# jmhb0/view_neti

Hardware: AMD Instinct MI355X
Metric: TI train steps/sec (SD-1.5 512^2 bs=4 per GPU) (higher is better)
Workload: dtype f16; 1 GPU; learnable_mode 0, sd15 shapes, 512x512 fp16, bs=4/GPU, grad_accum 1, full train step (VAE+16xCLIP+UNet fwd/bwd+AdamW); global_batch=4, parallelism=dp1, rccl_ranks=1, hipgraph=True

## Files before the change

include/vneti.h:

```cpp
#ifndef VNETI_H
#define VNETI_H
#include <stddef.h>
#include <stdint.h>

#ifdef __cplusplus
extern "C" {
#endif

#define VNETI_ABI_VERSION 1

int vneti_version(void);
int vneti_precision(void);
int vneti_last_error(char* buf, size_t n);

typedef struct vneti_gemm_desc {
  const void* A;
  const void* B;
  void* C;
  long long lda, ldb, ldc;
  int M, N, K;
  int batch;
  long long strideA, strideB, strideC;
  const float* bias;
  const void* rowadd;
// ... 1 lines not shown
  int rows_per_group;
  const void* resid;
  long long ldr;
  float alpha;
  int act;
  int out_f32;
  int conv_mode;
  int Hi, Wi, Ci, Ho, Wo, stride, pad_t, pad_l, ups;
  long long ldx;
  int tile_hint;
  void* workspace;
  long long workspace_bytes;
  int split_k;
  const void* gate_src;
  long long ld_gate;
  int gate_act;
  void* C2;
  long long ldc2;
  int act2;
  void* gn_sums;
  int gn_hw, gn_cpg, gn_groups, gn_slots;
  int geglu;
  int conv_korder;
} vneti_gemm_desc;

int vneti_gemm_f16(const vneti_gemm_desc* d, void* stream);
int vneti_gemm_select_tile(int M, int N, int batch);
int vneti_gemm_select_split(int M, int N, int K, int batch, int tile_hint, long long workspace_bytes);

int vneti_im2col3x3_small(const void* x, int x_is_f32, long long sb, long long sc, long long sy,
                          long long sx, void* out, int Bn, int C, int Hi, int Wi, int Ho, int Wo,
                          int stride, int pad_t, int pad_l, void* stream);

int vneti_conv3x3_in(const void* x, int x_is_f32, long long sb, long long sc, long long sy, long long sx,
                     const void* w_packed, const float* bias, void* out, long long ldo, int Bn, int C, int H, int W,
                     int Co, void* gn_sums, int gn_groups, int gn_slots, void* stream);

int vneti_transpose_f16(const void* in, long long ld_in, long long stride_in, void* out,
                        long long ld_out, long long stride_out, int rows, int cols, int batch,
                        void* stream);
#define VNETI_TRANSPOSE_MAX 4
typedef struct vneti_transpose_desc {
  const void* inp;
  long long ld_in, stride_in;
  void* out;
  long long ld_out, stride_out;
// ... 194 lines not shown
```

view_neti_amd/csrc/gemm_args.h:

```cpp
#pragma once
#include "common.h"

namespace {

struct GemmArgs {
  const half_t* A;
  const half_t* B;
  void* C;
  const float* bias;
  const half_t* rowadd;
  const void* resid;
  float* ws;
  const half_t* gate_src;
  half_t* C2;
  long long ld_gate, ldc2;
  int gate_act, act2;
  float* gn_sums;
  int gn_hw, gn_cpg, gn_G, gn_slots;
  int geglu;
  long long lda, ldb, ldc, ld_rowadd, ldr;
  long long strideA, strideB, strideC;
  uint32_t a_bytes, b_bytes;
  int M, N, K;
  int rows_per_group;
  float alpha;
  int act;
  int out_f32;
  int batch, ksplit, kt_per_split;
  int conv_mode;
  int Hi, Wi, Ci, Ho, Wo, stride, pad_t, pad_l, ups;
  int ldx2;
  int korder;
  int tiles_m, tiles_n;
};

__device__ __forceinline__ float apply_act(float v, int act) {
  switch (act) {
    case 1: return vn_silu(v);
    case 2: return vn_quick_gelu(v);
    case 3: return vn_gelu_erf(v);
    default: return v;
  }
}
__device__ __forceinline__ float act_grad(float f, int act) {
  if (act == 2) {
    float s = vn_sigmoid(1.702f * f);
    return s * (1.f + 1.702f * f * (1.f - s));
  } else if (act == 3) {
    return vn_gelu_erf_grad(f);
  }
  float s = vn_sigmoid(f);
  return s * (1.f + f * (1.f - s));
}

__device__ __forceinline__ int lds_off(int row, int chunk) {
  return row * 128 + ((chunk ^ ((row >> 1) & 7)) << 4);
}
// ... 13 lines not shown
```

view_neti_amd/csrc/gemm_conv.hip:

```cpp
#include "common.h"
#include "gemm_args.h"
#include "../../include/vneti.h"

namespace {

template <int BM, int BN, int WM, int WN, bool F32OUT, bool DMA, int NSTG = 2, int EPI = 2, bool CONV = true>
__global__ __launch_bounds__((BM / WM) * (BN / WN) * 64) void gemm_kernel(
    const half_t* pA, const half_t* pB, uint32_t p_a_bytes, uint32_t p_b_bytes, int p_lda, int p_ldb, int pM, int pN, int pK,
    int p_tiles_m, int p_tiles_n, int p_split_conv , const GemmArgs gfull) {
  GemmArgs g = gfull;
  g.A = pA;
  g.B = pB;
  g.a_bytes = p_a_bytes;
  g.b_bytes = p_b_bytes;
  g.lda = p_lda;
  g.ldb = p_ldb;
  g.M = pM;
  g.N = pN;
  g.K = pK;
  g.tiles_m = p_tiles_m;
  g.tiles_n = p_tiles_n;
  g.kt_per_split = p_split_conv & 0xffff;
  g.ksplit = (p_split_conv >> 16) & 0xff;
  g.conv_mode = p_split_conv >> 24;
  static_assert(NSTG == 2 || ((NSTG == 3 || NSTG == 4) && DMA), "the LDS rings are LDS-DMA only");
  const half_t* const e_gate = EPI == 2 ? g.gate_src : nullptr;
  half_t* const e_C2 = EPI == 2 ? g.C2 : nullptr;
  const int e_geglu = EPI == 2 ? g.geglu : 0;
  const int e_act = EPI == 2 ? g.act : 0;
  float* const e_gn_sums = EPI >= 1 ? g.gn_sums : nullptr;
  const half_t* const e_rowadd = EPI >= 1 ? g.rowadd : nullptr;
  const int e_conv = CONV ? g.conv_mode : 0;
  constexpr int NWM = BM / WM, NWN = BN / WN;
  constexpr int NT = NWM * NWN * 64;
  constexpr int RSTEP = NT / 8;
  constexpr int A_IT = BM / RSTEP, B_IT = BN / RSTEP;
  constexpr int STAGE_BYTES = (BM + BN) * 128;
  constexpr int CS_LD = F32OUT ? (BN + 4) : (BN + 8);
  constexpr int CS_BYTES = BM * CS_LD * (F32OUT ? 4 : 2);
  constexpr int LDS_BYTES = (NSTG * STAGE_BYTES > CS_BYTES) ? NSTG * STAGE_BYTES : CS_BYTES;
  constexpr int GN_IMG = 5, GN_NG = BN / 4 + 2;
  constexpr int GN_BYTES = (F32OUT || EPI == 0) ? 0 : GN_IMG * GN_NG * 4 * 8;
  __shared__ __attribute__((aligned(16))) char smem[LDS_BYTES + GN_BYTES];

  const int tid = threadIdx.x;
  const int lane = tid & 63;
  const int wave = __builtin_amdgcn_readfirstlane(tid >> 6);
  const int wm0 = (wave / NWN) * WM;
  const int wn0 = (wave % NWN) * WN;

  int nblk = g.tiles_m * g.tiles_n;
  int bid = blockIdx.x;
  {
    int q = nblk >> 3, r = nblk & 7, xcd = bid & 7, idx = bid >> 3;
    bid = (xcd < r ? xcd * (q + 1) : r * (q + 1) + (xcd - r) * q) + idx;
  }
  const int tile_m = bid / g.tiles_n;
  const int tile_n = bid - tile_m * g.tiles_n;
  const int m0 = tile_m * BM;
  const int n0 = tile_n * BN;
  const int bz = blockIdx.y;
  const int kz = blockIdx.z;

  const half_t* Ab = g.A + (long long)bz * g.strideA;
  const half_t* Bb = g.B + (long long)bz * g.strideB;
  __amdgpu_buffer_rsrc_t rsA = vn_make_rsrc(Ab, g.a_bytes);
  __amdgpu_buffer_rsrc_t rsB = vn_make_rsrc(Bb, g.b_bytes);

  const int lrow = tid >> 3;
  const int gchunk = DMA ? ((tid & 7) ^ ((lrow >> 1) & 7)) : (tid & 7);

  const float rcp_hw = CONV ? __builtin_amdgcn_rcpf((float)(g.Ho * g.Wo)) : 0.f, rcp_wo = CONV ? __builtin_amdgcn_rcpf((float)g.Wo) : 0.f;
  int a_off[A_IT];
  int a_py[A_IT], a_px[A_IT], a_bh[A_IT];
#pragma unroll
  for (int i = 0; i < A_IT; ++i) {
    int m = m0 + lrow + RSTEP * i;
    bool ok = m < g.M;
    if (e_conv == 0) {
      a_off[i] = ok ? (int)((long long)m * g.lda * 2) + gchunk * 16 : -1;
      a_py[i] = a_px[i] = a_bh[i] = 0;
    } else {
      int rem, ox;
      const int b = vn_divmod(m, g.Ho * g.Wo, rcp_hw, rem);
      const int oy = vn_divmod(rem, g.Wo, rcp_wo, ox);
      a_bh[i] = ok ? b * g.Hi : -1;
      if (e_conv == 1) {
        a_py[i] = oy * g.stride - g.pad_t;
        a_px[i] = ox * g.stride - g.pad_l;
      } else {
        a_py[i] = oy + g.pad_t;
        a_px[i] = ox + g.pad_l;
      }
      a_off[i] = ((b * g.Hi + a_py[i]) * g.Wi + a_px[i]) * g.ldx2 + gchunk * 16;
    }
  }
  int b_off[B_IT];
#pragma unroll
  for (int i = 0; i < B_IT; ++i) {
    int n = n0 + lrow + RSTEP * i;
    b_off[i] = (n < g.N) ? (int)((long long)n * g.ldb * 2) + gchunk * 16 : -1;
  }

  u32x4 ra[DMA ? 1 : A_IT], rb[DMA ? 1 : B_IT];

  auto a_offset = [&](int i, int k0, int dy, int dx, int tapoff) -> uint32_t {
    if (e_conv == 0) return a_off[i] < 0 ? VN_OOB : (uint32_t)(a_off[i] + k0 * 2);
    bool ok = a_bh[i] >= 0;
    if (e_conv == 1 && !g.ups) {
      int iy = a_py[i] + dy, ix = a_px[i] + dx;
      ok = ok && (unsigned)iy < (unsigned)g.Hi && (unsigned)ix < (unsigned)g.Wi;
      return ok ? (uint32_t)(a_off[i] + tapoff) : VN_OOB;
    }
    int iy, ix;
    if (e_conv == 1) {
// ... 18 lines not shown
  };

  uint32_t a_cur[A_IT], b_cur[B_IT];
#pragma unroll
  for (int i = 0; i < B_IT; ++i) b_cur[i] = b_off[i] < 0 ? VN_OOB : (uint32_t)b_off[i];

  auto issue = [&](int kt, int stage, bool first) {
    const int k0 = kt * 64;
    bool recompute = first;
    int dy = 0, dx = 0, tapoff = 0;
    if (e_conv != 0) {
      int tap, ci0;
      if (g.korder) {
        const int chunk = kt / 9;
        tap = kt - chunk * 9;
        ci0 = chunk << 6;
        recompute = true;
      } else {
        tap = k0 / g.Ci;
        ci0 = k0 - tap * g.Ci;
        recompute = recompute || ci0 == 0;
      }
      if (recompute) {
        dy = tap / 3;
        dx = tap - dy * 3;
        tapoff = (e_conv == 1 && !g.ups) ? ((dy * g.Wi + dx) * g.ldx2 + ci0 * 2) : (ci0 * 2 + gchunk * 16);
      }
    }
    if (recompute) {
#pragma unroll
      for (int i = 0; i < A_IT; ++i) a_cur[i] = a_offset(i, k0, dy, dx, tapoff);
      if (first) {
#pragma unroll
        for (int i = 0; i < B_IT; ++i) b_cur[i] += (uint32_t)k0 * 2;
      }
    }
    if constexpr (DMA) {
      char* As = smem + stage * STAGE_BYTES;
      char* Bs = As + BM * 128;
#pragma unroll
      for (int i = 0; i < A_IT; ++i) dma16(rsA, As + (wave * 8 + RSTEP * i) * 128, a_cur[i]);
#pragma unroll
      for (int i = 0; i < B_IT; ++i) dma16(rsB, Bs + (wave * 8 + RSTEP * i) * 128, b_cur[i]);
    } else {
#pragma unroll
      for (int i = 0; i < A_IT; ++i) ra[i] = vn_buf_load16(rsA, a_cur[i]);
#pragma unroll
      for (int i = 0; i < B_IT; ++i) rb[i] = vn_buf_load16(rsB, b_cur[i]);
// ... 238 lines not shown
          q_hi += __shfl_xor(q_hi, off);
        }
      }
      if (gn_img >= 0 && (!uni || lane < CPR)) {
        vn_u64* a = gacc + ((gn_img - gn_img0) * GN_NG + (gn_glo - gn_g0t)) * 4;
        vn_fx_add2(a, s_lo, q_lo);
        if (gn_split < 8) vn_fx_add2(a + 4, s_hi, q_hi);
      }
      s_lo = q_lo = s_hi = q_hi = 0.f;
    };
    for (int idx = tid; idx < BM * CPR; idx += NT) {
      int r = idx / CPR, c = (idx - r * CPR) * 8;
      int m = m0 + r, n = n0 + c;
      const bool valid = m < g.M && n < g.N;
      if (gn) {
        int gn_rem;
        const int img = valid ? vn_divmod(m, g.gn_hw, rcp_gnhw, gn_rem) : gn_img;
        if (__any(img != gn_img)) {
          gn_flush();
          gn_img = img;
        }
      }
      if (!valid) continue;
      half8 v = as_half8(*reinterpret_cast<const u32x4*>(smem + ((size_t)r * CS_LD + c) * 2));
      int ra_rem;
      const half_t* radd = e_rowadd ? e_rowadd + (long long)vn_divmod(m, g.rows_per_group, rcp_rpg, ra_rem) * g.ld_rowadd + n : nullptr;
      if (n + 8 <= g.N) {
        if (radd) {
          half8 t = *reinterpret_cast<const half8*>(radd);
          v = vn_add8(v, t);
        }
        if (Rb) {
          half8 rr = *reinterpret_cast<const half8*>(Rb + (long long)m * g.ldr + n);
          v = vn_add8(v, rr);
        }
        if (e_geglu == 2) {
          const half_t* pp = e_gate + (long long)m * g.ld_gate + 2 * n;
#pragma unroll
          for (int c2 = 0; c2 < 2; ++c2) {
            const half8 pre = *reinterpret_cast<const half8*>(pp + 8 * c2);
            half8 o;
#pragma unroll
            for (int e = 0; e < 4; ++e) {
              const float d = (float)v[4 * c2 + e], hh = (float)pre[e], gg = (float)pre[4 + e];
              float cdf, xpdf;
              vn_gelu_parts(gg, cdf, xpdf);
              o[e] = (half_t)(d * gg * cdf);
              o[4 + e] = (half_t)(d * hh * (cdf + xpdf));
            }
            vn_st16_wt(rsC, (uint32_t)(((long long)m * g.ldc + 2 * n + 8 * c2) * 2), o);
          }
          continue;
        }
        if (e_gate) {
          half8 pre = *reinterpret_cast<const half8*>(e_gate + (long long)m * g.ld_gate + n);
#pragma unroll
          for (int e = 0; e < 8; ++e) v[e] = (half_t)((float)v[e] * act_grad((float)pre[e], g.gate_act));
        }
        if (e_geglu == 1 || (e_C2 && e_geglu == 0)) vn_st16_wt_saved(rsC, (uint32_t)(((long long)m * g.ldc + n) * 2), v);
        else vn_st16_wt(rsC, (uint32_t)(((long long)m * g.ldc + n) * 2), v);
        if (e_geglu == 1) {
          half4 o2;
#pragma unroll
          for (int e = 0; e < 4; ++e) o2[e] = (half_t)((float)v[e] * vn_gelu_erf((float)v[4 + e]));
          *reinterpret_cast<half4*>(e_C2 + (long long)m * g.ldc2 + (n >> 1)) = o2;
        }
        if (gn) {
#pragma unroll
          for (int e = 0; e < 8; ++e) {
            const float x = (float)v[e];
            if (e < gn_split) {
              s_lo += x;
              q_lo += x * x;
            } else {
              s_hi += x;
              q_hi += x * x;
            }
          }
        }
        if (e_C2 && e_geglu == 0) {
          half8 o2;
#pragma unroll
          for (int e = 0; e < 8; ++e) o2[e] = (half_t)apply_act((float)v[e], g.act2);
          vn_st16_wt(rsC2, (uint32_t)(((long long)m * g.ldc2 + n) * 2), o2);
        }
      } else {
        for (int e = 0; e < 8 && n + e < g.N; ++e) {
          float x = (float)v[e];
          if (radd) x = (float)(half_t)(x + (float)radd[e]);
          if (Rb) x = (float)(half_t)(x + (float)Rb[(long long)m * g.ldr + n + e]);
          if (e_gate) x = (float)(half_t)(x * act_grad((float)e_gate[(long long)m * g.ld_gate + n + e], g.gate_act));
          Cb[(long long)m * g.ldc + n + e] = (half_t)x;
          if (e_C2) e_C2[(long long)m * g.ldc2 + n + e] = (half_t)apply_act((float)(half_t)x, g.act2);
          if (gn) {
            const float xs = (float)(half_t)x;
            if (e < gn_split) {
              s_lo += xs;
              q_lo += xs * xs;
            } else {
              s_hi += xs;
              q_hi += xs * xs;
            }
          }
        }
      }
    }
    if (gn) {
      gn_flush();
      __syncthreads();
      const int slot = tile_m % g.gn_slots;
      for (int i = tid; i < GN_IMG * GN_NG; i += NT) {
        const vn_u64* src = gacc + 4 * i;
        if ((src[0] | src[1] | src[2] | src[3]) == 0) continue;
        const int img = gn_img0 + i / GN_NG, grp = gn_g0t + i % GN_NG;
        vn_u64* dst = reinterpret_cast<vn_u64*>(e_gn_sums) + (((long long)img * g.gn_slots + slot) * g.gn_G + grp) * 4;
// ... 10 lines not shown
  GemmArgs g = gfull;
  g.ws = p_ws;
  g.C = pC;
  g.bias = p_bias;
  g.resid = p_resid;
  g.rowadd = p_rowadd;
  g.M = pM;
  g.N = pN;
  g.batch = p_batch;
  g.ksplit = p_ksplit;
  g.ldc = p_ldc;
  g.ldr = p_ldr;
  const unsigned n4 = (unsigned)(g.N + 3) / 4;
  const unsigned gid = blockIdx.x * 256u + threadIdx.x;
  const unsigned total = (unsigned)g.batch * (unsigned)g.M * n4;
  if (gid >= total) return;
  const unsigned row = gid / n4;
  const int c = (int)(gid - row * n4) * 4;
  const int bz = g.batch > 1 ? (int)(row / (unsigned)g.M) : 0;
  const int m = (int)(row - (unsigned)bz * (unsigned)g.M);
  const int ne = min(4, g.N - c);
  const long long zstride = (long long)g.batch * g.M * g.N;
  const float* p0 = g.ws + ((long long)bz * g.M + m) * g.N + c;
  if ((g.N & 3) == 0 && ((g.ldc | g.ldr | g.ld_rowadd | g.ld_gate | g.ldc2) & 3) == 0) {
    const long long co = (long long)bz * g.strideC + (long long)m * g.ldc + c;
    const long long ro = (long long)bz * g.strideC + (long long)m * g.ldr + c;
    f32x4 bv = {0.f, 0.f, 0.f, 0.f}, rf = {0.f, 0.f, 0.f, 0.f};
    half4 rh = {0, 0, 0, 0}, ra = {0, 0, 0, 0}, gt = {0, 0, 0, 0};
    if (g.bias) bv = *reinterpret_cast<const f32x4*>(g.bias + c);
    if (g.resid) {
      if (g.out_f32) rf = *reinterpret_cast<const f32x4*>(reinterpret_cast<const float*>(g.resid) + ro);
      else rh = *reinterpret_cast<const half4*>(reinterpret_cast<const half_t*>(g.resid) + ro);
    }
    if (g.rowadd) ra = *reinterpret_cast<const half4*>(g.rowadd + (long long)(m / g.rows_per_group) * g.ld_rowadd + c);
    if (g.gate_src) gt = *reinterpret_cast<const half4*>(g.gate_src + (long long)m * g.ld_gate + c);
    f32x4 v = {0.f, 0.f, 0.f, 0.f};
    int z = 0;
    for (; z + 4 <= g.ksplit; z += 4) {
      const f32x4 t0 = *reinterpret_cast<const f32x4*>(p0 + (z + 0) * zstride);
      const f32x4 t1 = *reinterpret_cast<const f32x4*>(p0 + (z + 1) * zstride);
      const f32x4 t2 = *reinterpret_cast<const f32x4*>(p0 + (z + 2) * zstride);
      const f32x4 t3 = *reinterpret_cast<const f32x4*>(p0 + (z + 3) * zstride);
      v += t0;
      v += t1;
      v += t2;
      v += t3;
    }
    for (; z < g.ksplit; ++z) v += *reinterpret_cast<const f32x4*>(p0 + z * zstride);
// ... 15 lines not shown
        float y = (float)(half_t)x[e];
        if (g.rowadd) y = (float)(half_t)(y + (float)ra[e]);
        if (g.resid) y = (float)(half_t)(y + (float)rh[e]);
        if (g.gate_src) y = (float)(half_t)(y * act_grad((float)gt[e], g.gate_act));
        o[e] = (half_t)y;
        o2[e] = (half_t)apply_act((float)(half_t)y, g.act2);
      }
      *reinterpret_cast<half4*>(reinterpret_cast<half_t*>(g.C) + co) = o;
      if (g.C2) *reinterpret_cast<half4*>(g.C2 + (long long)m * g.ldc2 + c) = o2;
    }
    return;
  }
  float v[4] = {0.f, 0.f, 0.f, 0.f};
  for (int z = 0; z < g.ksplit; ++z) {
    const float* p = p0 + z * zstride;
    for (int e = 0; e < ne; ++e) v[e] += p[e];
  }
  for (int e = 0; e < ne; ++e) {
    float x = v[e] * g.alpha;
    if (g.bias) x += g.bias[c + e];
    x = apply_act(x, g.act);
    if (g.out_f32) {
      if (g.resid) x += reinterpret_cast<const float*>(g.resid)[(long long)bz * g.strideC + (long long)m * g.ldr + c + e];
      reinterpret_cast<float*>(g.C)[(long long)bz * g.strideC + (long long)m * g.ldc + c + e] = x;
    } else {
      x = (float)(half_t)x;
      if (g.rowadd) x = (float)(half_t)(x + (float)g.rowadd[(long long)(m / g.rows_per_group) * g.ld_rowadd + c + e]);
      if (g.resid)
        x = (float)(half_t)(x + (float)reinterpret_cast<const half_t*>(g.resid)[(long long)bz * g.strideC + (long long)m * g.ldr + c + e]);
      if (g.gate_src) x = (float)(half_t)(x * act_grad((float)g.gate_src[(long long)m * g.ld_gate + c + e], g.gate_act));
      reinterpret_cast<half_t*>(g.C)[(long long)bz * g.strideC + (long long)m * g.ldc + c + e] = (half_t)x;
      if (g.C2) g.C2[(long long)m * g.ldc2 + c + e] = (half_t)apply_act((float)(half_t)x, g.act2);
    }
  }
}

inline int epilogue_level(const GemmArgs& g) {
  if (g.gate_src || g.C2 || g.geglu || g.act) return 2;
  return (g.gn_sums || g.rowadd) ? 1 : 0;
}

template <int BM, int BN, int WM, int WN, bool F32OUT, bool DMA, int NSTG>
void launch_variant(const GemmArgs& g, dim3 grid, hipStream_t st) {
  const dim3 block((BM / WM) * (BN / WN) * 64);
#define VN_GO(E, C)                                                                                                        \
  hipLaunchKernelGGL((gemm_kernel<BM, BN, WM, WN, F32OUT, DMA, NSTG, E, C>), grid, block, 0, st, g.A, g.B, g.a_bytes, g.b_bytes, \
                     (int)g.lda, (int)g.ldb, g.M, g.N, g.K, g.tiles_m, g.tiles_n, g.kt_per_split | (g.ksplit << 16) | (g.conv_mode << 24), g)
  if constexpr (F32OUT) {
    if (g.conv_mode) { if (g.act) VN_GO(2, true); else VN_GO(0, true); }
    else { if (g.act) VN_GO(2, false); else VN_GO(0, false); }
  } else {
    const int epi = epilogue_level(g);
    if (g.conv_mode) { if (epi == 2) VN_GO(2, true); else if (epi == 1) VN_GO(1, true); else VN_GO(0, true); }
    else { if (epi == 2) VN_GO(2, false); else if (epi == 1) VN_GO(1, false); else VN_GO(0, false); }
// ... 115 lines not shown
  g.gn_G = d->gn_groups;
  g.gn_slots = d->gn_slots;
  g.geglu = d->geglu;
  g.lda = d->lda;
  g.ldb = d->ldb;
  g.ldc = d->ldc;
  g.ld_rowadd = d->ld_rowadd;
  g.ldr = d->ldr;
  g.strideA = d->strideA;
  g.strideB = d->strideB;
  g.strideC = d->strideC;
  g.M = d->M;
  g.N = d->N;
  g.K = d->K;
  g.batch = batch;
  g.rows_per_group = d->rows_per_group > 0 ? d->rows_per_group : 1;
  g.alpha = d->alpha;
  g.act = d->act;
  g.out_f32 = d->out_f32 ? 1 : 0;
  g.conv_mode = d->conv_mode;
  long long a_bytes;
  if (d->conv_mode == 0) {
    VN_REQUIRE(d->lda % 8 == 0, "gemm: lda=%lld must be a multiple of 8", d->lda);
    a_bytes = ((long long)(d->M - 1) * d->lda + d->K) * 2;
  } else {
    VN_REQUIRE(d->conv_mode == 1 || d->conv_mode == 2, "gemm: bad conv_mode %d", d->conv_mode);
    VN_REQUIRE(d->Ci > 0 && d->Ci % 64 == 0, "conv: Ci=%d must be a multiple of 64", d->Ci);
    VN_REQUIRE(d->K == 9 * d->Ci, "conv: K=%d must equal 9*Ci=%d", d->K, 9 * d->Ci);
    VN_REQUIRE(d->stride == 1 || d->stride == 2, "conv: stride %d unsupported", d->stride);
    VN_REQUIRE(d->Ho > 0 && d->Wo > 0 && d->M % (d->Ho * d->Wo) == 0, "conv: M=%d not a multiple of Ho*Wo", d->M);
    VN_REQUIRE(d->ldx % 8 == 0, "conv: ldx must be a multiple of 8");
    VN_REQUIRE(!(d->ups && d->conv_mode != 1), "conv: fused upsample only in forward gather mode");
    VN_REQUIRE(!(d->ups && d->stride != 1), "conv: fused upsample needs stride 1");
    g.Hi = d->Hi;
    g.Wi = d->Wi;
    g.Ci = d->Ci;
    g.Ho = d->Ho;
    g.Wo = d->Wo;
    g.stride = d->stride;
    g.pad_t = d->pad_t;
    g.pad_l = d->pad_l;
    g.ups = d->ups;
    g.ldx2 = (int)(d->ldx * 2);
    VN_REQUIRE(!d->conv_korder || d->Ci % 64 == 0, "conv: conv_korder=1 needs Ci=%d to be a multiple of 64", d->Ci);
    g.korder = d->conv_korder ? 1 : 0;
    long long nb = d->M / (d->Ho * d->Wo);
    a_bytes = nb * d->Hi * d->Wi * d->ldx * 2;
  }
  long long b_bytes = ((long long)(d->N - 1) * d->ldb + d->K) * 2;
  VN_REQUIRE(a_bytes < 0x7fffffffLL && b_bytes < 0x7fffffffLL, "gemm: operand larger than 2 GiB");
  g.a_bytes = (uint32_t)a_bytes;
  g.b_bytes = (uint32_t)b_bytes;
  if (!d->out_f32) {
    VN_REQUIRE(d->ldc % 8 == 0 || d->N < 8, "gemm: ldc=%lld must be a multiple of 8", d->ldc);
  }
  VN_REQUIRE_OUT("gemm C", vn_out_bytes(d->M, d->ldc, d->N, d->out_f32 ? 4 : 2, batch, d->strideC));
  if (d->C2) VN_REQUIRE_OUT("gemm C2", vn_out_bytes(d->M, d->ldc2, d->geglu == 1 ? d->N / 2 : d->N, 2));
  hipStream_t st = (hipStream_t)stream;
  bool f32 = d->out_f32 != 0;
  VN_REQUIRE(!(f32 && d->rowadd), "gemm: rowadd is only supported for f16 output");
  if (d->gate_src || d->C2) {
    VN_REQUIRE(!f32 && batch == 1, "gemm: gate/C2 epilogues need f16 output and batch 1");
    VN_REQUIRE(!d->gate_src || (d->gate_act >= 1 && d->gate_act <= 3 && d->ld_gate % 8 == 0), "gemm: bad gate arguments");
    VN_REQUIRE(!d->C2 || (d->act2 >= 0 && d->act2 <= 3 && d->ldc2 % 8 == 0), "gemm: bad C2 arguments");
  }

  if (d->geglu) {
    VN_REQUIRE(d->geglu == 1 || d->geglu == 2, "gemm: geglu must be 0, 1 or 2");
    VN_REQUIRE(!f32 && batch == 1 && d->N % 8 == 0, "gemm: geglu needs f16 output, batch 1 and N %% 8 == 0");
    VN_REQUIRE(d->split_k == 1, "gemm: geglu needs split_k = 1 (it lives in the fused epilogue)");
    VN_REQUIRE(!d->gn_sums, "gemm: geglu and gn_sums are exclusive");
    if (d->geglu == 1) {
      VN_REQUIRE(d->C2 && d->ldc2 % 4 == 0 && !d->gate_src, "gemm: geglu forward needs C2 ([M][N/2]) and no gate");
    } else {
      VN_REQUIRE(d->gate_src && d->ld_gate % 8 == 0 && !d->C2 && !d->resid && !d->rowadd,
                 "gemm: geglu backward needs gate_src ([M][2N] saved pre-activation) and a plain epilogue");
      VN_REQUIRE(d->ldc % 8 == 0, "gemm: geglu backward writes [M][2N]: ldc %% 8");
    }
  }
  if (d->gn_sums) {
    VN_REQUIRE(!f32 && batch == 1, "gemm: gn_sums needs f16 output and batch 1");
    VN_REQUIRE(d->gn_hw >= 64 && d->gn_cpg >= 4 && d->gn_groups > 0 && d->gn_slots > 0 && d->N == d->gn_cpg * d->gn_groups &&
                   d->M % d->gn_hw == 0 && (d->gn_cpg >= 8 || d->gn_cpg == 4),
               "gemm: bad gn_sums geometry hw=%d cpg=%d G=%d", d->gn_hw, d->gn_cpg, d->gn_groups);
    VN_REQUIRE(d->split_k == 1, "gemm: gn_sums needs split_k = 1 (the statistics live in the fused epilogue)");
  }

  int cfg = d->tile_hint;
  bool dma = true;
  if (cfg >= 100) {
    dma = false;
    cfg -= 100;
  }
  if (cfg == 0) cfg = select_tile(d->M, d->N, batch);
  VN_REQUIRE(cfg >= 1 && cfg <= kMaxTile, "gemm: unknown tile_hint %d", d->tile_hint);
  if (cfg == 18 &&
      (d->conv_mode < 1 || d->conv_mode > 2 || d->stride != 1 || d->ups || d->pad_t != 1 || d->pad_l != 1 || d->Hi != d->Ho ||
       d->Wi != d->Wo || (d->Ho & 15) || (d->Wo & 15) || (d->Ci & 63) || !d->conv_korder || batch != 1 || f32))
    cfg = 17;
  if (cfg == 18 && d->gn_sums && (d->gn_cpg & 1)) cfg = 17;
  if ((cfg == 16 || cfg == 17) && (!dma || (d->conv_mode && (d->ups || (d->conv_mode == 2 && d->stride == 2))) ||
                    (d->gn_sums && (d->gn_cpg & 1)) ||
                    (d->M >= (1 << 24) && (d->conv_mode || d->rowadd || d->gn_sums)))) cfg = cfg == 16 ? 5 : 7;
  if ((cfg == 5 || cfg == 16) && f32) cfg = 4;
  if (cfg == 17 && f32) cfg = 7;
  if ((cfg == 6 || cfg == 7) && !dma) cfg = 4;
  if (cfg >= 10 && !dma) cfg = kTiles[cfg].bm == 128 ? (kTiles[cfg].bn == 128 ? 1 : 2) : 3;
  long long ws_floats = d->workspace ? d->workspace_bytes / 4 : 0;
  int ks = d->split_k;
  if (ks == 0) ks = select_ksplit(d->M, d->N, d->K, batch, cfg, ws_floats);
  if (ks < 1) ks = 1;
  const int nk = d->K / 64;
  if (ks > nk) ks = nk;
  if (ks > 1) {
    VN_REQUIRE(d->workspace && (long long)ks * batch * d->M * d->N <= ws_floats,
               "gemm: split_k=%d needs %lld workspace bytes", ks, (long long)ks * batch * d->M * d->N * 4);
    VN_REQUIRE(batch == 1 || (d->strideC != 0), "gemm: batched split-K needs strideC");
    VN_REQUIRE((long long)batch * d->M * ((d->N + 3) / 4) < 0x7fffffffLL, "gemm: split-K output larger than 2^31 chunks");
    VN_REQUIRE_OUT("gemm split-K workspace", (long long)ks * batch * d->M * d->N * 4);
  }
  if (cfg == 18 && ks > d->Ci / 64) ks = d->Ci / 64;
  g.ksplit = ks;
  g.kt_per_split = cdiv(nk, ks);
  g.ksplit = cdiv(nk, g.kt_per_split);
  VN_REQUIRE(g.ksplit <= 255 && g.kt_per_split <= 0xffff, "gemm: split_k=%d / K=%d out of range", g.ksplit, d->K);
  g.ws = (float*)d->workspace;

#define LAUNCH(BM, BN, WM, WN) \
  return dma ? launch_cfg<BM, BN, WM, WN, true>(g, f32, st) : launch_cfg<BM, BN, WM, WN, false>(g, f32, st)
  switch (cfg) {
    case 1: LAUNCH(128, 128, 64, 64);
    case 2: LAUNCH(128, 64, 64, 32);
    case 3: LAUNCH(64, 64, 32, 32);
    case 4: LAUNCH(256, 128, 64, 64);
    case 6: return launch_cfg_ring<256, 128, 64, 64>(g, f32, st);
    case 7: return launch_cfg_ring<256, 128, 64, 32>(g, f32, st);
    case 8: LAUNCH(256, 128, 64, 32);
    case 9: LAUNCH(128, 128, 64, 32);
    case 10: return launch_cfg_ring<128, 128, 64, 32>(g, f32, st);
    case 11: return launch_cfg_ring<128, 64, 64, 32>(g, f32, st);
// ... 18 lines not shown
```

view_neti_amd/engine/schedule.py:

```python
from __future__ import annotations

from functools import partial
from typing import Dict, List

import torch

from .. import lib, ops, packing


class T:

    __slots__ = ("v", "g", "gw", "rows", "cols", "children", "need_grad", "producer")

    def __init__(self, v, g=None, need_grad=True):
        self.v = v
        self.g = g
        self.gw = False
        self.rows, self.cols = v.shape
        self.children: List["T"] = []
        self.need_grad = need_grad
        self.producer = None


def rup(x, m):
# ... 74 lines not shown
    def _contrib_gemm(self, t: T, A, Bm, **kw):
        g = self._grad(t)
        resid = g if t.gw else None
        self.bwd.append(partial(ops.gemm, A, Bm, g, resid=resid, **kw))
        if not t.gw:
            t.gw = True
            for c in t.children:
                c.gw = True

    _tile_cache: Dict[tuple, int] = {}
    _TILE_DIMS = {1: (128, 128), 2: (128, 64), 3: (64, 64), 4: (256, 128), 5: (256, 256), 6: (256, 128), 7: (256, 128),
                  8: (256, 128), 9: (128, 128), 10: (128, 128), 11: (128, 64), 12: (64, 64), 13: (128, 128), 14: (128, 64),
                  15: (64, 64), 16: (256, 256), 17: (256, 128), 18: (256, 128)}

    @staticmethod
    def _gemm_key(f):
        kw = f.keywords
        A, Bm, out = f.args[:3]
        conv = kw.get("conv")
        M = kw.get("M") or A.shape[-2]
        N = kw.get("N") or Bm.shape[-2]
        K = kw.get("K") or Bm.shape[-1]
        ck = (conv["mode"], conv["stride"], conv["ups"], conv["Hi"], conv["Wi"]) if conv else None
        return (M, N, K, kw.get("batch") or 1, ck, out.dtype == torch.float32, kw.get("geglu") or 0)

    def autotune(self, candidates=(1, 2, 3, 5, 6, 7, 8, 9, 10, 11, 12, 13, 14, 15, 16, 17, 18), reps=8):
        if not torch.cuda.is_available():
            return
        import json
        import os
        from .. import parallel
        if os.environ.get("VNETI_AUTOTUNE_CANDS"):
            candidates = tuple(int(x) for x in os.environ["VNETI_AUTOTUNE_CANDS"].split(","))
        how = _timing_switches(self.dev, reps)
        cache = Schedule._tile_cache
        cache_path = os.environ.get("VNETI_AUTOTUNE_CACHE")
        if cache_path and os.path.exists(cache_path) and not cache:
            cache.update(picks_from_json(json.load(open(cache_path))))
        n_before = len(cache)
        share = parallel.sharing_picks() and parallel._dist() is not None
        rank0 = (not share) or parallel._dist().get_rank() == 0
        if share and not rank0:
            cache.update(parallel.share_from_rank0(None))
        for lst in (self.fwd_pre, self.fwd, self.bwd):
            for idx, f in enumerate(lst):
                if getattr(f, "func", None) is not ops.gemm or f.keywords.get("tile_hint"):
# ... 246 lines not shown
        x, out, Cc, h, wd = r["x"], r["out"], r["C"], r["h"], r["wd"]
        assert out.gw
        desc = self._conv_desc(h // 2, wd // 2, Cc, h, wd, 2, r["pad"], 0, out.g.stride(0), mode=2)
        self._contrib_gemm(x, out.g, r["wd_"], M=x.rows, conv=desc)

    def forward_pre(self):
        for f in self.fwd_pre:
            f()

    def forward_main(self):
        for f in self.fwd:
            f()

    def forward(self):
        self.forward_pre()
        self.forward_main()

    def backward(self):
        for f in self.bwd:
            f()


def _chunk_major_ok(conv) -> bool:
    return bool(conv) and not conv.get("ups") and not conv.get("korder") and \
        not (conv["mode"] == 2 and conv["stride"] == 2) and conv["Ci"] % 64 == 0 and conv["Ci"] >= 128


def gemm_variants(key, conv, geglu, candidates) -> List[tuple]:
    M, N, K, batch = key[:4]
    try_cm = _chunk_major_ok(conv)
    halo_ok = try_cm and conv["mode"] in (1, 2) and conv["stride"] == 1 and conv["pad_t"] == 1 and conv["pad_l"] == 1 \
        and conv["Ho"] % 16 == 0 and conv["Wo"] % 16 == 0 and conv["Hi"] == conv["Ho"] and conv["Wi"] == conv["Wo"]
    tiles_ko = [(h, 0) for h in candidates if h != 18] + \
        ([(h, 1) for h in candidates if h in (16, 17) or (h == 18 and halo_ok)] if try_cm else [])
    out = []
    for h, ko in tiles_ko:
        bm, bn = Schedule._TILE_DIMS[h]
        tiles = -(-M // bm) * -(-N // bn) * batch
        sks = (0, 1) + (tuple(x for x in (2, 3, 4, 6, 8, 12)
                              if x * 8 <= K // 64 and tiles * x <= 1024 and x * batch * M * N <= 16 * 2 ** 20)
                        if tiles < 256 else ())
        if geglu:
            sks = (1,)
        out += [(h, sk, ko) for sk in sks]
    return out


def _timing_switches(dev, reps):
    import os
    cold = None if os.environ.get("VNETI_AUTOTUNE_HOT") else torch.empty(160 * 2 ** 20, dtype=torch.float32, device=dev)
    return (cold, reps, int(os.environ.get("VNETI_AUTOTUNE_REPS", "9")),
            bool(int(os.environ.get("VNETI_AUTOTUNE_WARM_A", "1"))))


def _time_call(call, act, cold, reps, cold_reps, warm_a):
# ... 44 lines not shown
```

view_neti_amd/engine/unet.py:

```python
from __future__ import annotations

from functools import partial
from typing import Dict

import torch

from .. import ops, packing
from .. import sd_config as sc
from .schedule import Schedule, T, rup as _rup


class UNetEngine(Schedule):
    def __init__(self, cfg: sc.UNetConfig, weights: Dict[str, torch.Tensor], batch: int, height: int, width: int,
                 ctx_len: int = 77, device: str = "cuda", need_backward: bool = True, autotune: bool = True,
                 fuse_gn: bool = True):
        super().__init__(batch, cfg.norm_num_groups, cfg.norm_eps, device, need_backward)
        self.cfg = cfg
        self.H, self.W = height, width
        self.L = ctx_len
        self.nl = cfg.n_cross_layers
        B, L, Dc = batch, ctx_len, cfg.cross_attention_dim
        self.x_in = self._buf((B, cfg.in_channels, height, width), torch.float32)
        self.timesteps = torch.zeros(B, dtype=torch.int64, device=device)
        self.ctx_k = self._buf((self.nl, B * L, Dc))
        self.ctx_v = self._buf((self.nl, B * L, Dc))
        self.dctx_k = self._buf((self.nl, B * L, Dc))
        self.dctx_v = self._buf((self.nl, B * L, Dc))
        self.pred = self._buf((B * height * width, 8))[:, : cfg.out_channels]
        self.dpred = self._buf((B * height * width, 8), zero=True)[:, : cfg.out_channels]
        self._pack_time_weights(weights)
        self._plan_kv()
        self._build(weights)
        self._kv_fwd_ops()
        if need_backward:
            self._build_backward()
            self._kv_bwd_ops()
        if autotune:
            self.autotune()
        self.bind_workspace()
        self.fuse_gn_stats(fuse=fuse_gn)
# ... 183 lines not shown
        bw.append(partial(ops.gemm, dq2, r["wq2d"], dn2))
        dh1 = self._tmp("tF", M, Cc)
        bw.append(partial(self._ln_bwd, r["ln2"], dn2, dh1, dh2))
        do1 = self._tmp("tA", M, Cc)
        bw.append(partial(ops.gemm, dh1, r["wo1d"], do1))
        qkv = r["qkv"]
        q, k, v = qkv[:, :Cc], qkv[:, Cc:2 * Cc], qkv[:, 2 * Cc:]
        dqkv = self._tmp("tC", M, 3 * Cc)
        dq, dk, dv = dqkv[:, :Cc], dqkv[:, Cc:2 * Cc], dqkv[:, 2 * Cc:]
        bw.append(partial(ops.attn_bwd_dq, q, k, v, do1, r["lse1"], delta, dq, B, heads, N, N, D, r["scale"], False,
                          O=r["o1"]))
        bw.append(partial(ops.attn_bwd_dkv, q, k, v, do1, r["lse1"], delta, dk, dv, B, heads, N, N, D, r["scale"],
                          False))
        dn1 = self._tmp("tD", M, Cc)
        bw.append(partial(ops.gemm, dqkv, r["wqkvd"], dn1))
        dh0 = self._tmp("tE", M, Cc)
        bw.append(partial(self._ln_bwd, r["ln1"], dn1, dh0, dh1))
        dg = self._tmp("tA", M, Cc)
        bw.append(partial(ops.gemm, dh0, r["w_ind"], dg))
        self._contrib(x, self._gn_bwd_fn(r["gn"], dg), extra=dout)

    def _upsample(self, x: T, Cc, name, w, out_view, h, wd):
        M = x.rows * 4
        wf = self._w16(packing.conv3x3_fwd(w[name + "weight"]))
        b = self._w32(w[name + "bias"])
        out = T(out_view if out_view is not None else self._buf((M, Cc)))
        self.fwd.append(partial(ops.gemm, x.v, wf, out.v, bias=b, M=M,
                                conv=self._conv_desc(h, wd, Cc, 2 * h, 2 * wd, 1, 1, 1, x.v.stride(0))))
        self._produced(out)
        rec = dict(kind="up", x=x, out=out, C=Cc, h=h, wd=wd)
        if self.need_backward:
            rec["wd_"] = self._w16(packing.conv3x3_dgrad(w[name + "weight"]))
        self.tape.append(rec)
        return out

    def _upsample_bwd(self, r):
        x, out, Cc, h, wd = r["x"], r["out"], r["C"], r["h"], r["wd"]
        assert out.gw and not x.gw
        M = out.rows
        dup = self._tmp("dA", M, Cc)
        self.bwd.append(partial(ops.gemm, out.g, r["wd_"], dup, M=M,
                                conv=self._conv_desc(2 * h, 2 * wd, Cc, 2 * h, 2 * wd, 1, 1, 0, out.g.stride(0), mode=2)))
        g = self._grad(x)
        self.bwd.append(partial(ops.sum2x2, dup, g, self.B, h, wd, Cc))
        x.gw = True

    def _build(self, w):
        cfg = self.cfg
        B, H, W = self.B, self.H, self.W
        boc = cfg.block_out_channels
        nlev = len(boc)
        nres = cfg.layers_per_block + 1
        self._time_ops()
        catT = {}
        for i in range(nlev):
            lvl = nlev - 1 - i
            m = B * (H >> lvl) * (W >> lvl)
            for j in range(nres):
                rin, skip, _ = sc.up_block_channels(cfg, i, j)
                catT[(i, j)] = T(self._buf((m, rin + skip)),
                                 self._buf((m, rin + skip)) if self.need_backward else None)

# ... 123 lines not shown
```

view_neti_amd/ops.py:

```python
from __future__ import annotations

import ctypes as C

import torch

from . import lib as _l

ACT_NONE, ACT_SILU, ACT_QUICK_GELU, ACT_GELU = 0, 1, 2, 3


def stream() -> int:
    return torch.cuda.current_stream().cuda_stream


def _p(t):
    return None if t is None else t.data_ptr()


def _ld(t):
    if t is None:
        return 0
    assert t.stride(-1) == 1, "last dim must be contiguous"
    return t.stride(-2) if t.dim() >= 2 else t.shape[-1]

# ... 7 lines not shown


def gemm(A, B, out, *, bias=None, rowadd=None, rows_per_group=1, resid=None, alpha=1.0, act=0,
         tile_hint=0, batch=0, strideA=0, strideB=0, strideC=0, M=None, N=None, K=None, conv=None,
         lda=None, ldc=None, workspace=None, split_k=0, gate=None, gate_act=0, out2=None, act2=0,
         gn_sums=None, gn_hw=0, gn_groups=0, gn_slots=0, geglu=0):
    d = _l.GemmDesc()
    d.A, d.B, d.C = _p(A), _p(B), _p(out)
    d.ldb = _ld(B)
    d.ldc = ldc if ldc is not None else _ld(out)
    d.N = N if N is not None else B.shape[-2]
    d.K = K if K is not None else B.shape[-1]
    if conv is None:
        d.M = M if M is not None else A.shape[-2]
        d.lda = lda if lda is not None else _ld(A)
        d.conv_mode = 0
    else:
        d.M = M
        d.lda = 0
        d.conv_mode = conv["mode"]
        for k in ("Hi", "Wi", "Ci", "Ho", "Wo", "stride", "pad_t", "pad_l", "ups", "ldx"):
            setattr(d, k, int(conv.get(k, 0)))
        d.conv_korder = int(conv.get("korder", 0))
    d.batch = batch
    d.strideA, d.strideB, d.strideC = strideA, strideB, strideC
    d.bias = _p(bias)
    d.rowadd = _p(rowadd)
    d.ld_rowadd = _ld(rowadd) if rowadd is not None else 0
    d.rows_per_group = rows_per_group
    d.resid = _p(resid)
    d.ldr = _ld(resid) if resid is not None else 0
    d.alpha = alpha
    d.act = act
    d.out_f32 = 1 if out.dtype == torch.float32 else 0
    d.tile_hint = tile_hint
    if gate is not None:
        d.gate_src, d.ld_gate, d.gate_act = _p(gate), _ld(gate), gate_act
    if out2 is not None:
        d.C2, d.ldc2, d.act2 = _p(out2), _ld(out2), act2
    if gn_sums is not None:
        d.gn_sums, d.gn_hw, d.gn_groups, d.gn_slots = _p(gn_sums), gn_hw, gn_groups, gn_slots
        d.gn_cpg = d.N // gn_groups
    d.geglu = geglu
    ws = workspace if workspace is not None else _default_ws
    if ws is not None:
        d.workspace = ws.data_ptr()
# ... 423 lines not shown
```

view_neti_amd/packing.py:

```python
from __future__ import annotations

import os

import torch

KORDER_CM = os.environ.get("VNETI_CONV_KORDER", "0") == "1"


def _chunk_major(m: torch.Tensor, n_out: int, c: int) -> torch.Tensor:
    return m.reshape(n_out, 9, c // 64, 64).permute(0, 2, 1, 3).reshape(n_out, 9 * c).contiguous()


def conv3x3_fwd(w: torch.Tensor, cm=None) -> torch.Tensor:
    co, ci, kh, kw = w.shape
    assert kh == 3 and kw == 3
    m = w.permute(0, 2, 3, 1).reshape(co, 9 * ci).contiguous()
    cm = KORDER_CM if cm is None else cm
    return _chunk_major(m, co, ci) if cm and ci % 64 == 0 else m


def conv3x3_dgrad(w: torch.Tensor, cm=None) -> torch.Tensor:
    co, ci, kh, kw = w.shape
    assert kh == 3 and kw == 3
    m = w.permute(1, 2, 3, 0).reshape(ci, 9 * co).contiguous()
    cm = KORDER_CM if cm is None else cm
    return _chunk_major(m, ci, co) if cm and co % 64 == 0 else m


def pad_rows(w: torch.Tensor, mult: int) -> torch.Tensor:
    k = w.shape[-1]
    kp = (k + mult - 1) // mult * mult
    if kp == k:
        return w.contiguous()
    out = torch.zeros(*w.shape[:-1], kp, dtype=w.dtype, device=w.device)
    out[..., :k] = w
    return out


def geglu_interleave_index(n2: int, device=None) -> torch.Tensor:
    F = n2 // 2
    assert n2 % 8 == 0
    r = torch.arange(n2, device=device)
    q, e = r // 8, r % 8
    return torch.where(e < 4, 4 * q + e, F + 4 * q + e - 4)


def geglu_interleave(w: torch.Tensor) -> torch.Tensor:
    return w[geglu_interleave_index(w.shape[0], w.device)].contiguous()

# ... 13 lines not shown
```

Before: 39.82 steps/s.

## Collapse nearest-upsample + 3x3 conv into four 2x2 phase convolutions

Replaces the UNet upsample conv (nearest 2x upsample followed by a 3x3 conv) with four per-phase 2x2 convolutions on the low-resolution input. Their weights are pre-summed, and each phase writes its output rows interleaved into the full-resolution buffer. The backward data gradient becomes a single stride-2 4x4 conv, which removes the temporary full-resolution dgrad buffer and the reduction that followed it. This cuts conv FLOPs from 9 to 4 taps per output (forward) and avoids work on the upsampled input. In exchange, these layers lose the fast halo/chunk-major tile configs 16-18, and the summed weights in fp16 slightly change the numerics.

```diff
diff --git a/include/vneti.h b/include/vneti.h
--- a/include/vneti.h
+++ b/include/vneti.h
@@ -47,6 +47,8 @@
   int gn_hw, gn_cpg, gn_groups, gn_slots;
   int geglu;
   int conv_korder;
+  int conv_kh, conv_kw;
+  int ups_phase;
 } vneti_gemm_desc;
 
 int vneti_gemm_f16(const vneti_gemm_desc* d, void* stream);
diff --git a/view_neti_amd/csrc/gemm_args.h b/view_neti_amd/csrc/gemm_args.h
--- a/view_neti_amd/csrc/gemm_args.h
+++ b/view_neti_amd/csrc/gemm_args.h
@@ -32,7 +32,16 @@
   int ldx2;
   int korder;
   int tiles_m, tiles_n;
+  int kw;
+  int phase;
 };
+
+__device__ __forceinline__ int vn_c_row(int m, int phase, int z, int Wo, float rcp_wo) {
+  if (!phase) return m;
+  int j;
+  const int r = vn_divmod(m, Wo, rcp_wo, j);
+  return (2 * r + (z >> 1)) * 2 * Wo + 2 * j + (z & 1);
+}
 
 __device__ __forceinline__ float apply_act(float v, int act) {
   switch (act) {
diff --git a/view_neti_amd/csrc/gemm_conv.hip b/view_neti_amd/csrc/gemm_conv.hip
--- a/view_neti_amd/csrc/gemm_conv.hip
+++ b/view_neti_amd/csrc/gemm_conv.hip
@@ -31,6 +31,7 @@
   float* const e_gn_sums = EPI >= 1 ? g.gn_sums : nullptr;
   const half_t* const e_rowadd = EPI >= 1 ? g.rowadd : nullptr;
   const int e_conv = CONV ? g.conv_mode : 0;
+  const int e_phase = CONV ? g.phase : 0;
   constexpr int NWM = BM / WM, NWN = BN / WN;
   constexpr int NT = NWM * NWN * 64;
   constexpr int RSTEP = NT / 8;
@@ -73,6 +74,7 @@
   const float rcp_hw = CONV ? __builtin_amdgcn_rcpf((float)(g.Ho * g.Wo)) : 0.f, rcp_wo = CONV ? __builtin_amdgcn_rcpf((float)g.Wo) : 0.f;
   int a_off[A_IT];
   int a_py[A_IT], a_px[A_IT], a_bh[A_IT];
+  const int pad_t = e_phase ? 1 - (bz >> 1) : g.pad_t, pad_l = e_phase ? 1 - (bz & 1) : g.pad_l;
 #pragma unroll
   for (int i = 0; i < A_IT; ++i) {
     int m = m0 + lrow + RSTEP * i;
@@ -86,11 +88,11 @@
       const int oy = vn_divmod(rem, g.Wo, rcp_wo, ox);
       a_bh[i] = ok ? b * g.Hi : -1;
       if (e_conv == 1) {
-        a_py[i] = oy * g.stride - g.pad_t;
-        a_px[i] = ox * g.stride - g.pad_l;
+        a_py[i] = oy * g.stride - pad_t;
+        a_px[i] = ox * g.stride - pad_l;
       } else {
-        a_py[i] = oy + g.pad_t;
-        a_px[i] = ox + g.pad_l;
+        a_py[i] = oy + pad_t;
+        a_px[i] = ox + pad_l;
       }
       a_off[i] = ((b * g.Hi + a_py[i]) * g.Wi + a_px[i]) * g.ldx2 + gchunk * 16;
     }
@@ -155,8 +157,8 @@
         recompute = recompute || ci0 == 0;
       }
       if (recompute) {
-        dy = tap / 3;
-        dx = tap - dy * 3;
+        dy = g.kw == 3 ? tap / 3 : (g.kw == 2 ? tap >> 1 : tap >> 2);
+        dx = tap - dy * g.kw;
         tapoff = (e_conv == 1 && !g.ups) ? ((dy * g.Wi + dx) * g.ldx2 + ci0 * 2) : (ci0 * 2 + gchunk * 16);
       }
     }
@@ -441,6 +443,7 @@
         }
       }
       if (!valid) continue;
+      const int mc = vn_c_row(m, e_phase, bz, g.Wo, rcp_wo);
       half8 v = as_half8(*reinterpret_cast<const u32x4*>(smem + ((size_t)r * CS_LD + c) * 2));
       int ra_rem;
       const half_t* radd = e_rowadd ? e_rowadd + (long long)vn_divmod(m, g.rows_per_group, rcp_rpg, ra_rem) * g.ld_rowadd + n : nullptr;
@@ -477,7 +480,7 @@
           for (int e = 0; e < 8; ++e) v[e] = (half_t)((float)v[e] * act_grad((float)pre[e], g.gate_act));
         }
         if (e_geglu == 1 || (e_C2 && e_geglu == 0)) vn_st16_wt_saved(rsC, (uint32_t)(((long long)m * g.ldc + n) * 2), v);
-        else vn_st16_wt(rsC, (uint32_t)(((long long)m * g.ldc + n) * 2), v);
+        else vn_st16_wt(rsC, (uint32_t)(((long long)mc * g.ldc + n) * 2), v);
         if (e_geglu == 1) {
           half4 o2;
 #pragma unroll
@@ -509,7 +512,7 @@
           if (radd) x = (float)(half_t)(x + (float)radd[e]);
           if (Rb) x = (float)(half_t)(x + (float)Rb[(long long)m * g.ldr + n + e]);
           if (e_gate) x = (float)(half_t)(x * act_grad((float)e_gate[(long long)m * g.ld_gate + n + e], g.gate_act));
-          Cb[(long long)m * g.ldc + n + e] = (half_t)x;
+          Cb[(long long)mc * g.ldc + n + e] = (half_t)x;
           if (e_C2) e_C2[(long long)m * g.ldc2 + n + e] = (half_t)apply_act((float)(half_t)x, g.act2);
           if (gn) {
             const float xs = (float)(half_t)x;
@@ -566,8 +569,9 @@
   const int ne = min(4, g.N - c);
   const long long zstride = (long long)g.batch * g.M * g.N;
   const float* p0 = g.ws + ((long long)bz * g.M + m) * g.N + c;
+  const int mc = g.phase ? vn_c_row(m, 1, bz, g.Wo, __builtin_amdgcn_rcpf((float)g.Wo)) : m;
   if ((g.N & 3) == 0 && ((g.ldc | g.ldr | g.ld_rowadd | g.ld_gate | g.ldc2) & 3) == 0) {
-    const long long co = (long long)bz * g.strideC + (long long)m * g.ldc + c;
+    const long long co = (long long)bz * g.strideC + (long long)mc * g.ldc + c;
     const long long ro = (long long)bz * g.strideC + (long long)m * g.ldr + c;
     f32x4 bv = {0.f, 0.f, 0.f, 0.f}, rf = {0.f, 0.f, 0.f, 0.f};
     half4 rh = {0, 0, 0, 0}, ra = {0, 0, 0, 0}, gt = {0, 0, 0, 0};
@@ -629,14 +633,14 @@
     x = apply_act(x, g.act);
     if (g.out_f32) {
       if (g.resid) x += reinterpret_cast<const float*>(g.resid)[(long long)bz * g.strideC + (long long)m * g.ldr + c + e];
-      reinterpret_cast<float*>(g.C)[(long long)bz * g.strideC + (long long)m * g.ldc + c + e] = x;
+      reinterpret_cast<float*>(g.C)[(long long)bz * g.strideC + (long long)mc * g.ldc + c + e] = x;
     } else {
       x = (float)(half_t)x;
       if (g.rowadd) x = (float)(half_t)(x + (float)g.rowadd[(long long)(m / g.rows_per_group) * g.ld_rowadd + c + e]);
       if (g.resid)
         x = (float)(half_t)(x + (float)reinterpret_cast<const half_t*>(g.resid)[(long long)bz * g.strideC + (long long)m * g.ldr + c + e]);
       if (g.gate_src) x = (float)(half_t)(x * act_grad((float)g.gate_src[(long long)m * g.ld_gate + c + e], g.gate_act));
-      reinterpret_cast<half_t*>(g.C)[(long long)bz * g.strideC + (long long)m * g.ldc + c + e] = (half_t)x;
+      reinterpret_cast<half_t*>(g.C)[(long long)bz * g.strideC + (long long)mc * g.ldc + c + e] = (half_t)x;
       if (g.C2) g.C2[(long long)m * g.ldc2 + c + e] = (half_t)apply_act((float)(half_t)x, g.act2);
     }
   }
@@ -798,11 +802,24 @@
   long long a_bytes;
   if (d->conv_mode == 0) {
     VN_REQUIRE(d->lda % 8 == 0, "gemm: lda=%lld must be a multiple of 8", d->lda);
+    VN_REQUIRE(!d->conv_kh && !d->conv_kw && !d->ups_phase, "gemm: conv_kh / conv_kw / ups_phase need conv_mode 1");
     a_bytes = ((long long)(d->M - 1) * d->lda + d->K) * 2;
   } else {
     VN_REQUIRE(d->conv_mode == 1 || d->conv_mode == 2, "gemm: bad conv_mode %d", d->conv_mode);
     VN_REQUIRE(d->Ci > 0 && d->Ci % 64 == 0, "conv: Ci=%d must be a multiple of 64", d->Ci);
-    VN_REQUIRE(d->K == 9 * d->Ci, "conv: K=%d must equal 9*Ci=%d", d->K, 9 * d->Ci);
+    const int kh = d->conv_kh ? d->conv_kh : 3, kw = d->conv_kw ? d->conv_kw : 3;
+    VN_REQUIRE(kh == kw && (kh == 3 || ((kh == 2 || kh == 4) && d->conv_mode == 1 && !d->ups && !d->conv_korder)),
+               "conv: tap grid %dx%d unsupported (3x3; 2x2 / 4x4 in conv_mode 1 without ups and with conv_korder 0)", kh, kw);
+    VN_REQUIRE(d->K == kh * kw * d->Ci, "conv: K=%d must equal %d*Ci=%d", d->K, kh * kw, kh * kw * d->Ci);
+    g.kw = kw;
+    if (d->ups_phase) {
+      VN_REQUIRE(d->ups_phase == 1 && kh == 2 && d->stride == 1 && d->Hi == d->Ho && d->Wi == d->Wo && batch == 4 &&
+                     d->strideA == 0 && d->strideC == 0,
+                 "conv: ups_phase needs 2x2 taps, stride 1, Hi x Wi = Ho x Wo, batch 4 and strideA = strideC = 0");
+      VN_REQUIRE(!d->out_f32 && !d->resid && !d->rowadd && !d->gate_src && !d->C2 && !d->geglu && !d->gn_sums,
+                 "conv: ups_phase takes bias / act only (f16 output)");
+      g.phase = 1;
+    }
     VN_REQUIRE(d->stride == 1 || d->stride == 2, "conv: stride %d unsupported", d->stride);
     VN_REQUIRE(d->Ho > 0 && d->Wo > 0 && d->M % (d->Ho * d->Wo) == 0, "conv: M=%d not a multiple of Ho*Wo", d->M);
     VN_REQUIRE(d->ldx % 8 == 0, "conv: ldx must be a multiple of 8");
@@ -830,7 +847,8 @@
   if (!d->out_f32) {
     VN_REQUIRE(d->ldc % 8 == 0 || d->N < 8, "gemm: ldc=%lld must be a multiple of 8", d->ldc);
   }
-  VN_REQUIRE_OUT("gemm C", vn_out_bytes(d->M, d->ldc, d->N, d->out_f32 ? 4 : 2, batch, d->strideC));
+  if (g.phase) VN_REQUIRE_OUT("gemm C", vn_out_bytes(4LL * d->M, d->ldc, d->N, 2));
+  else VN_REQUIRE_OUT("gemm C", vn_out_bytes(d->M, d->ldc, d->N, d->out_f32 ? 4 : 2, batch, d->strideC));
   if (d->C2) VN_REQUIRE_OUT("gemm C2", vn_out_bytes(d->M, d->ldc2, d->geglu == 1 ? d->N / 2 : d->N, 2));
   hipStream_t st = (hipStream_t)stream;
   bool f32 = d->out_f32 != 0;
@@ -875,7 +893,7 @@
        d->Wi != d->Wo || (d->Ho & 15) || (d->Wo & 15) || (d->Ci & 63) || !d->conv_korder || batch != 1 || f32))
     cfg = 17;
   if (cfg == 18 && d->gn_sums && (d->gn_cpg & 1)) cfg = 17;
-  if ((cfg == 16 || cfg == 17) && (!dma || (d->conv_mode && (d->ups || (d->conv_mode == 2 && d->stride == 2))) ||
+  if ((cfg == 16 || cfg == 17) && (!dma || (d->conv_mode && (d->ups || (d->conv_mode == 2 && d->stride == 2) || g.kw != 3 || g.phase)) ||
                     (d->gn_sums && (d->gn_cpg & 1)) ||
                     (d->M >= (1 << 24) && (d->conv_mode || d->rowadd || d->gn_sums)))) cfg = cfg == 16 ? 5 : 7;
   if ((cfg == 5 || cfg == 16) && f32) cfg = 4;
@@ -891,7 +909,7 @@
   if (ks > 1) {
     VN_REQUIRE(d->workspace && (long long)ks * batch * d->M * d->N <= ws_floats,
                "gemm: split_k=%d needs %lld workspace bytes", ks, (long long)ks * batch * d->M * d->N * 4);
-    VN_REQUIRE(batch == 1 || (d->strideC != 0), "gemm: batched split-K needs strideC");
+    VN_REQUIRE(batch == 1 || (d->strideC != 0) || g.phase, "gemm: batched split-K needs strideC");
     VN_REQUIRE((long long)batch * d->M * ((d->N + 3) / 4) < 0x7fffffffLL, "gemm: split-K output larger than 2^31 chunks");
     VN_REQUIRE_OUT("gemm split-K workspace", (long long)ks * batch * d->M * d->N * 4);
   }
diff --git a/view_neti_amd/engine/schedule.py b/view_neti_amd/engine/schedule.py
--- a/view_neti_amd/engine/schedule.py
+++ b/view_neti_amd/engine/schedule.py
@@ -120,6 +120,8 @@
         N = kw.get("N") or Bm.shape[-2]
         K = kw.get("K") or Bm.shape[-1]
         ck = (conv["mode"], conv["stride"], conv["ups"], conv["Hi"], conv["Wi"]) if conv else None
+        if conv and _other_taps(conv):
+            ck += (conv.get("kh", 0), conv.get("kw", 0), conv.get("phase", 0))
         return (M, N, K, kw.get("batch") or 1, ck, out.dtype == torch.float32, kw.get("geglu") or 0)
 
     def autotune(self, candidates=(1, 2, 3, 5, 6, 7, 8, 9, 10, 11, 12, 13, 14, 15, 16, 17, 18), reps=8):
@@ -412,8 +414,12 @@
 
 
 def _chunk_major_ok(conv) -> bool:
-    return bool(conv) and not conv.get("ups") and not conv.get("korder") and \
+    return bool(conv) and not conv.get("ups") and not conv.get("korder") and not _other_taps(conv) and \
         not (conv["mode"] == 2 and conv["stride"] == 2) and conv["Ci"] % 64 == 0 and conv["Ci"] >= 128
+
+
+def _other_taps(conv) -> bool:
+    return bool(conv.get("kh") or conv.get("kw") or conv.get("phase"))
 
 
 def gemm_variants(key, conv, geglu, candidates) -> List[tuple]:
@@ -421,6 +427,8 @@
     try_cm = _chunk_major_ok(conv)
     halo_ok = try_cm and conv["mode"] in (1, 2) and conv["stride"] == 1 and conv["pad_t"] == 1 and conv["pad_l"] == 1 \
         and conv["Ho"] % 16 == 0 and conv["Wo"] % 16 == 0 and conv["Hi"] == conv["Ho"] and conv["Wi"] == conv["Wo"]
+    if conv and _other_taps(conv):
+        candidates = [h for h in candidates if h not in (16, 17, 18)]
     tiles_ko = [(h, 0) for h in candidates if h != 18] + \
         ([(h, 1) for h in candidates if h in (16, 17) or (h == 18 and halo_ok)] if try_cm else [])
     out = []
diff --git a/view_neti_amd/engine/unet.py b/view_neti_amd/engine/unet.py
--- a/view_neti_amd/engine/unet.py
+++ b/view_neti_amd/engine/unet.py
@@ -13,9 +13,10 @@
 class UNetEngine(Schedule):
     def __init__(self, cfg: sc.UNetConfig, weights: Dict[str, torch.Tensor], batch: int, height: int, width: int,
                  ctx_len: int = 77, device: str = "cuda", need_backward: bool = True, autotune: bool = True,
-                 fuse_gn: bool = True):
+                 fuse_gn: bool = True, collapse_ups: bool = True):
         super().__init__(batch, cfg.norm_num_groups, cfg.norm_eps, device, need_backward)
         self.cfg = cfg
+        self.collapse_ups = collapse_ups
         self.H, self.W = height, width
         self.L = ctx_len
         self.nl = cfg.n_cross_layers
@@ -245,15 +246,21 @@
 
     def _upsample(self, x: T, Cc, name, w, out_view, h, wd):
         M = x.rows * 4
-        wf = self._w16(packing.conv3x3_fwd(w[name + "weight"]))
         b = self._w32(w[name + "bias"])
         out = T(out_view if out_view is not None else self._buf((M, Cc)))
-        self.fwd.append(partial(ops.gemm, x.v, wf, out.v, bias=b, M=M,
-                                conv=self._conv_desc(h, wd, Cc, 2 * h, 2 * wd, 1, 1, 1, x.v.stride(0))))
+        if self.collapse_ups:
+            wf = self._w16(packing.conv3x3_ups_fwd(w[name + "weight"]))
+            conv = dict(self._conv_desc(h, wd, Cc, h, wd, 1, 1, 0, x.v.stride(0)), korder=0, kh=2, kw=2, phase=1)
+            self.fwd.append(partial(ops.gemm, x.v, wf[0], out.v, bias=b, M=x.rows, batch=4, strideB=wf[0].numel(), conv=conv))
+        else:
+            wf = self._w16(packing.conv3x3_fwd(w[name + "weight"]))
+            self.fwd.append(partial(ops.gemm, x.v, wf, out.v, bias=b, M=M,
+                                    conv=self._conv_desc(h, wd, Cc, 2 * h, 2 * wd, 1, 1, 1, x.v.stride(0))))
         self._produced(out)
         rec = dict(kind="up", x=x, out=out, C=Cc, h=h, wd=wd)
         if self.need_backward:
-            rec["wd_"] = self._w16(packing.conv3x3_dgrad(w[name + "weight"]))
+            pack = packing.conv3x3_ups_dgrad if self.collapse_ups else packing.conv3x3_dgrad
+            rec["wd_"] = self._w16(pack(w[name + "weight"]))
         self.tape.append(rec)
         return out
 
@@ -261,6 +268,11 @@
         x, out, Cc, h, wd = r["x"], r["out"], r["C"], r["h"], r["wd"]
         assert out.gw and not x.gw
         M = out.rows
+        if self.collapse_ups:
+            conv = dict(self._conv_desc(2 * h, 2 * wd, Cc, h, wd, 2, 1, 0, out.g.stride(0)), korder=0, kh=4, kw=4)
+            self.bwd.append(partial(ops.gemm, out.g, r["wd_"], self._grad(x), M=x.rows, conv=conv))
+            x.gw = True
+            return
         dup = self._tmp("dA", M, Cc)
         self.bwd.append(partial(ops.gemm, out.g, r["wd_"], dup, M=M,
                                 conv=self._conv_desc(2 * h, 2 * wd, Cc, 2 * h, 2 * wd, 1, 1, 0, out.g.stride(0), mode=2)))
diff --git a/view_neti_amd/ops.py b/view_neti_amd/ops.py
--- a/view_neti_amd/ops.py
+++ b/view_neti_amd/ops.py
@@ -53,6 +53,7 @@
         for k in ("Hi", "Wi", "Ci", "Ho", "Wo", "stride", "pad_t", "pad_l", "ups", "ldx"):
             setattr(d, k, int(conv.get(k, 0)))
         d.conv_korder = int(conv.get("korder", 0))
+        d.conv_kh, d.conv_kw, d.ups_phase = int(conv.get("kh", 0)), int(conv.get("kw", 0)), int(conv.get("phase", 0))
     d.batch = batch
     d.strideA, d.strideB, d.strideC = strideA, strideB, strideC
     d.bias = _p(bias)
diff --git a/view_neti_amd/packing.py b/view_neti_amd/packing.py
--- a/view_neti_amd/packing.py
+++ b/view_neti_amd/packing.py
@@ -25,6 +25,27 @@
     m = w.permute(1, 2, 3, 0).reshape(ci, 9 * co).contiguous()
     cm = KORDER_CM if cm is None else cm
     return _chunk_major(m, ci, co) if cm and co % 64 == 0 else m
+
+
+def _ups_collapsed(w: torch.Tensor) -> torch.Tensor:
+    co, ci, kh, kw = w.shape
+    assert kh == 3 and kw == 3
+    R = torch.tensor([[[1, 0, 0], [0, 1, 1]], [[1, 1, 0], [0, 0, 1]]], dtype=torch.float64, device=w.device)
+    return torch.einsum("aty,oiyx,bsx->aboits", R, w.to(torch.float64), R)
+
+
+def conv3x3_ups_fwd(w: torch.Tensor) -> torch.Tensor:
+    co, ci = w.shape[:2]
+    wc = _ups_collapsed(w)
+    return wc.permute(0, 1, 2, 4, 5, 3).reshape(4, co, 4 * ci).contiguous()
+
+
+def conv3x3_ups_dgrad(w: torch.Tensor) -> torch.Tensor:
+    co, ci = w.shape[:2]
+    wc = _ups_collapsed(w)
+    a_of, t_of = (1, 0, 1, 0), (1, 1, 0, 0)
+    rows = [wc[a_of[u], a_of[v], :, :, t_of[u], t_of[v]] for u in range(4) for v in range(4)]
+    return torch.stack(rows, 0).permute(2, 0, 1).reshape(ci, 16 * co).contiguous()
 
 
 def pad_rows(w: torch.Tensor, mult: int) -> torch.Tensor:
```

New measurement: 40.14 steps/s (median of 6 runs). About the same (+0.8%).
